# Modalities/modalities

Measured on AMD Instinct MI355X. Metric: train_tokens_per_s, higher is better.
Workload: dtype bf16; 1 GPU; model=gpt2-2.7b, global_batch=2, micro_batch=2, seq_len=4096, parallelism=dp1_fullshard_hipgraph, num_params=2795276800

## Files before the change

### modalities_amd/models/gpt2.py

```python

import math
from enum import Enum
from typing import Annotated, Optional

import torch
import torch.nn as nn
from pydantic import BaseModel, Field, model_validator

from modalities_amd.models.model import NNModel, SwiGLU
from modalities_amd.ops import flash_attention, precompute_rope_cos_sin, rope_apply
from modalities_amd.exceptions import ConfigError
from modalities_amd.ops.attention import (DECODE_HEAD_DIMS, _doc_visible,
                                          decode_attention,
                                          decode_attention_enabled,
                                          decode_rope_append, document_starts,
                                          fused_qkv_rope_attention)
from modalities_amd.ops.backend import use_hip
from modalities_amd.ops.layer_norm import LayerNorm
from modalities_amd.ops.linear import TwoStreamLinear
from modalities_amd.ops.rms_norm import RMSNorm


class PositionTypes(str, Enum):
    ABSOLUTE = "ABSOLUTE"
    NOPE = "NOPE"


class AttentionImplementation(str, Enum):
    HIP_FLASH = "hip_flash"
    PYTORCH_FLASH = "pytorch_flash"
    MANUAL = "manual"


class ActivationType(str, Enum):
    GELU = "gelu"
    SWIGLU = "swiglu"


class QueryKeyValueTransformType(str, Enum):
    ROTARY = "RotaryTransform"
    IDENTITY = "IdentityTransform"


class LayerNormVariant(str, Enum):
    RMS_NORM = "rms_norm"
    LAYER_NORM = "layer_norm"


class LayerNormConfig(BaseModel):
    variant: LayerNormVariant = LayerNormVariant.RMS_NORM
    eps: float = 1e-6
    bias: bool = True

# ... 215 lines not shown
            att = att.masked_fill(~mask, float("-inf")).softmax(-1)
            y = att @ vt
        return y.transpose(1, 2)


class TransformerMLP(nn.Module):
    def __init__(self, n_embd: int, ffn_hidden: int, bias: bool, dropout: float):
        super().__init__()
        self.c_fc = TwoStreamLinear(n_embd, ffn_hidden, bias=bias)
        self.gelu = nn.GELU(approximate="tanh")
        self.c_proj = TwoStreamLinear(ffn_hidden, n_embd, bias=bias)
        self.dropout = nn.Dropout(dropout)

    def forward(self, x):
        return self.dropout(self.c_proj(self.gelu(self.c_fc(x))))


class GPT2Block(nn.Module):

    def __init__(self, cfg: GPT2LLMConfig):
        super().__init__()
        self.attention_norm = make_norm(cfg.attention_norm_config, cfg.n_embd)
        self.attn = CausalSelfAttention(
            cfg.n_embd, cfg.n_head_q, cfg.n_head_kv, cfg.bias, cfg.dropout,
            cfg.attention_implementation, cfg.use_qk_norm,
            cfg.attention_norm_config, fused_qkv=cfg.fused_qkv)
        self.ffn_norm = make_norm(cfg.ffn_norm_config, cfg.n_embd)
        if cfg.activation_type == ActivationType.SWIGLU:
            self.mlp = SwiGLU(cfg.n_embd, cfg.ffn_hidden, cfg.bias,
                              packed=cfg.packed_swiglu)
        else:
            self.mlp = TransformerMLP(cfg.n_embd, cfg.ffn_hidden, cfg.bias, cfg.dropout)

    def forward(self, x, rope_cos, rope_sin, doc_start=None):
        if doc_start is None:
            x = x + self.attn(self.attention_norm(x), rope_cos, rope_sin)
        else:
            x = x + self.attn(self.attention_norm(x), rope_cos, rope_sin,
                              doc_start=doc_start)
        x = x + self.mlp(self.ffn_norm(x))
        return x

    def forward_cached(self, x, rope_cos, rope_sin, cache_k, cache_v, pos,
                       dec=None):
        if dec is None:
            x = x + self.attn.forward_cached(self.attention_norm(x), rope_cos,
                                             rope_sin, cache_k, cache_v, pos)
        else:
            x = x + self.attn.forward_cached(self.attention_norm(x), rope_cos,
                                             rope_sin, cache_k, cache_v, pos,
                                             dec=dec)
        x = x + self.mlp(self.ffn_norm(x))
        return x


class GPT2LLM(NNModel):
    def __init__(self, config: GPT2LLMConfig):
        if isinstance(config, dict):
            config = GPT2LLMConfig(**config)
        weight_decay_groups = {
            "linear": [r"attn\..*attn\.weight", r"attn\.qkv_attn\.weight",
                       r"attn\.c_proj\.weight",
                       r"mlp\..*\.weight", r"lm_head\.weight"],
            "embedding": [r"wte\.weight", r"wpe\.weight"],
            "norm": [r"norm", r"ln_", r"\.bias"],
        }
        super().__init__(seed=config.seed, weight_decay_groups=weight_decay_groups)
# ... 134 lines not shown
```

### modalities_amd/ops/csrc/bindings.cpp

```cpp
#include <torch/extension.h>

std::vector<torch::Tensor> rmsnorm_fwd(torch::Tensor x, torch::Tensor w, double eps);
std::vector<torch::Tensor> rmsnorm_bwd(torch::Tensor dy, torch::Tensor x,
                                       torch::Tensor w, torch::Tensor invrms);
std::vector<torch::Tensor> layernorm_fwd(torch::Tensor x, torch::Tensor w,
                                         c10::optional<torch::Tensor> b,
                                         double eps);
std::vector<torch::Tensor> layernorm_bwd(torch::Tensor dy, torch::Tensor x,
                                         torch::Tensor w, torch::Tensor mean,
                                         torch::Tensor rstd, bool has_bias);
long layernorm_max_h();
torch::Tensor rope_fwd(torch::Tensor x, torch::Tensor cos_t, torch::Tensor sin_t,
                       bool neg);
torch::Tensor rope_fwd_slice(torch::Tensor qkv, torch::Tensor cos_t,
                             torch::Tensor sin_t, long col_off, long Hn,
                             long D, bool neg);
void rope_bwd_slice(torch::Tensor dx, torch::Tensor cos_t, torch::Tensor sin_t,
                    torch::Tensor dqkv, long col_off);
torch::Tensor silu_mul_fwd(torch::Tensor g, torch::Tensor u);
std::vector<torch::Tensor> silu_mul_bwd(torch::Tensor dout, torch::Tensor g,
                                        torch::Tensor u);
torch::Tensor silu_mul_joint_fwd(torch::Tensor wv);
torch::Tensor silu_mul_joint_bwd(torch::Tensor dout, torch::Tensor wv);
std::vector<torch::Tensor> cross_entropy_fwd(torch::Tensor logits,
                                             torch::Tensor targets,
                                             long ignore_index);
torch::Tensor cross_entropy_bwd(torch::Tensor logits, torch::Tensor targets,
                                torch::Tensor lse, torch::Tensor scale,
                                long ignore_index);
void fused_adamw_masked(torch::Tensor p, torch::Tensor g, torch::Tensor m,
                        torch::Tensor v, torch::Tensor wd_mask, double lr,
                        double beta1, double beta2, double eps, double wd,
                        double bc1, double bc2);
void fused_adamw_masked_devstep(torch::Tensor p, torch::Tensor g,
                                torch::Tensor m, torch::Tensor v,
                                torch::Tensor wd_mask, torch::Tensor step,
                                torch::Tensor bf16_out,
// ... 61 lines not shown
                                         torch::Tensor k, torch::Tensor v,
                                         torch::Tensor o, torch::Tensor lse,
                                         bool causal, long q_offset,
                                         torch::Tensor doc_start,
                                         torch::Tensor doc_end,
                                         c10::optional<torch::Tensor> dlse);
std::vector<torch::Tensor> attn_bwd2_qkvjoint_doc(
    torch::Tensor dout, torch::Tensor q, torch::Tensor k, torch::Tensor v,
    torch::Tensor o, torch::Tensor lse, bool causal, long q_offset,
    torch::Tensor doc_start, torch::Tensor doc_end, torch::Tensor dqkv,
    long dv_col_off);
std::vector<torch::Tensor> decode_attn_fwd(torch::Tensor q,
                                           torch::Tensor k_cache,
                                           torch::Tensor v_cache,
                                           torch::Tensor kv_lens,
                                           long kv_chunk);
long decode_attn_kv_chunk();
long decode_attn_kv_chunk_min();
torch::Tensor decode_rope_append(torch::Tensor q, torch::Tensor k,
                                 torch::Tensor v,
                                 c10::optional<torch::Tensor> cos_t,
                                 c10::optional<torch::Tensor> sin_t,
                                 torch::Tensor pos, torch::Tensor k_cache,
                                 torch::Tensor v_cache);

static int g_attn_impl = [] {
  const char* e = getenv("MA_ATTN_IMPL");
  return e ? atoi(e) : 2;
}();

PYBIND11_MODULE(TORCH_EXTENSION_NAME, m) {
  m.def("rmsnorm_fwd", &rmsnorm_fwd, "RMSNorm forward (K5)");
  m.def("rmsnorm_bwd", &rmsnorm_bwd, "RMSNorm backward (K5)");
  m.def("layernorm_fwd", &layernorm_fwd,
        "LayerNorm forward (K5): (y, mean, rstd); b may be None",
        py::arg("x"), py::arg("w"), py::arg("b"), py::arg("eps"));
  m.def("layernorm_bwd", &layernorm_bwd,
        "LayerNorm backward (K5): (dx, dw, db); db is empty without bias",
        py::arg("dy"), py::arg("x"), py::arg("w"), py::arg("mean"),
        py::arg("rstd"), py::arg("has_bias"));
  m.def("layernorm_max_h", &layernorm_max_h,
        "largest row length the LayerNorm kernels take");
  m.def("rope_fwd", &rope_fwd, "RoPE rotate-half (K4); neg=true => inverse");
  m.def("rope_fwd_slice", &rope_fwd_slice,
        "RoPE a head-block slice of fused QKV into a contiguous [B,T,H,D]");
  m.def("rope_bwd_slice", &rope_bwd_slice,
        "inverse-RoPE a [B,T,H,D] grad into a fused-QKV grad buffer slice");
  m.def("silu_mul_fwd", &silu_mul_fwd, "silu(g)*u forward (K6)");
  m.def("silu_mul_bwd", &silu_mul_bwd, "silu(g)*u backward (K6)");
  m.def("silu_mul_joint_fwd", &silu_mul_joint_fwd,
        "silu/mul over a packed [.., 2H] gate|up tensor (K6 joint)");
  m.def("silu_mul_joint_bwd", &silu_mul_joint_bwd,
        "joint-layout silu/mul backward into one dwv buffer");
  m.def("cross_entropy_fwd", &cross_entropy_fwd, "fused CE forward (K8)");
  m.def("cross_entropy_bwd", &cross_entropy_bwd, "fused CE backward (K8)");
  m.def("fused_adamw_masked", &fused_adamw_masked,
        "AdamW on a flat fp32 shard with per-element wd mask (K9)");
  m.def("fused_adamw", &fused_adamw, "multi-tensor AdamW (K9)");
  m.def("fused_adamw_masked_devstep", &fused_adamw_masked_devstep,
        "AdamW with device-resident step counter (hipGraph-safe)");
  m.def("multi_tensor_sqsum", &multi_tensor_sqsum, "sum of squares (K10)");
  m.def("fused_adamw_devstep_bf16g", &fused_adamw_devstep_bf16g,
        "device-step AdamW reading a bf16 grad (* gmul) and a bit-packed "
        "decay mask (K9)");
  m.def("multi_tensor_sqsum_bf16", &multi_tensor_sqsum_bf16,
        "sum of squares of float(bf16) * gmul (K10)");
// ... 126 lines not shown
```

### modalities_amd/ops/csrc/rms_norm.hip

```cpp
#include <torch/extension.h>
#include <ATen/hip/HIPContext.h>
#include "common.h"

namespace {

constexpr int BLOCK = 256;

__global__ void rmsnorm_fwd_kernel(const unsigned short* __restrict__ x,
                                   const unsigned short* __restrict__ w,
                                   unsigned short* __restrict__ y,
                                   float* __restrict__ invrms,
                                   int H, float eps) {
  __shared__ float scratch[BLOCK / WAVE_SIZE];
  const long row = blockIdx.x;
  const unsigned short* xr = x + row * (long)H;
  unsigned short* yr = y + row * (long)H;

  float ss = 0.f;
  const int vecH = (H % 8 == 0) ? H / 8 : 0;
  const shortx8* xv = reinterpret_cast<const shortx8*>(xr);
  for (int i = threadIdx.x; i < vecH; i += BLOCK) {
    shortx8 v = xv[i];
#pragma unroll
    for (int j = 0; j < 8; ++j) {
      float f = bf16_to_f32((unsigned short)v[j]);
      ss += f * f;
    }
  }
  for (int i = vecH * 8 + threadIdx.x; i < H; i += BLOCK) {
    float f = bf16_to_f32(xr[i]);
    ss += f * f;
  }
  ss = block_reduce_sum(ss, scratch);
  const float r = rsqrtf(ss / H + eps);
  if (threadIdx.x == 0) invrms[row] = r;

  const shortx8* wv = reinterpret_cast<const shortx8*>(w);
  shortx8* yv = reinterpret_cast<shortx8*>(yr);
  for (int i = threadIdx.x; i < vecH; i += BLOCK) {
    shortx8 xvv = xv[i], wvv = wv[i], o;
#pragma unroll
    for (int j = 0; j < 8; ++j) {
      float f = bf16_to_f32((unsigned short)xvv[j]) * r *
                bf16_to_f32((unsigned short)wvv[j]);
      o[j] = (short)f32_to_bf16(f);
    }
    yv[i] = o;
  }
  for (int i = vecH * 8 + threadIdx.x; i < H; i += BLOCK) {
    yr[i] = f32_to_bf16(bf16_to_f32(xr[i]) * r * bf16_to_f32(w[i]));
  }
}

template <int SLOTS>
__global__ void rmsnorm_bwd_kernel(const unsigned short* __restrict__ dy,
                                   const unsigned short* __restrict__ x,
                                   const unsigned short* __restrict__ w,
                                   const float* __restrict__ invrms,
                                   unsigned short* __restrict__ dx,
                                   float* __restrict__ dw,
                                   int H, long N, int rows_per_block) {
  extern __shared__ __attribute__((aligned(16))) char smem_raw[];
  float* slab = reinterpret_cast<float*>(smem_raw);
  const int nwaves = blockDim.x / WAVE_SIZE;
  const int lane = threadIdx.x & (WAVE_SIZE - 1);
  const int wid = threadIdx.x / WAVE_SIZE;
  float* my_slab = slab + (long)wid * H;

  const long row0 = (long)blockIdx.x * rows_per_block;
  const long row1 = min(row0 + rows_per_block, N);
  const int vecH = H / 8;

  float dwacc[SLOTS][8];
#pragma unroll
  for (int it = 0; it < SLOTS; ++it)
#pragma unroll
    for (int j = 0; j < 8; ++j) dwacc[it][j] = 0.f;

  const shortx8* wv = reinterpret_cast<const shortx8*>(w);
  for (long row = row0 + wid; row < row1; row += nwaves) {
    const shortx8* xv = reinterpret_cast<const shortx8*>(x + row * (long)H);
    const shortx8* dyv = reinterpret_cast<const shortx8*>(dy + row * (long)H);
    shortx8* dxv = reinterpret_cast<shortx8*>(dx + row * (long)H);
    const float r = invrms[row];

    float dot = 0.f;
#pragma unroll
    for (int it = 0; it < SLOTS; ++it) {
      const int i = lane + it * WAVE_SIZE;
      if (i < vecH) {
        shortx8 xvv = xv[i], dyvv = dyv[i], wvv = wv[i];
#pragma unroll
        for (int j = 0; j < 8; ++j) {
          dot += bf16_to_f32((unsigned short)dyvv[j]) *
                 bf16_to_f32((unsigned short)wvv[j]) *
                 bf16_to_f32((unsigned short)xvv[j]);
        }
      }
    }
    dot = wave_reduce_sum(dot);
    const float k = r * r * r * dot / H;

#pragma unroll
    for (int it = 0; it < SLOTS; ++it) {
      const int i = lane + it * WAVE_SIZE;
      if (i < vecH) {
        shortx8 xvv = xv[i], dyvv = dyv[i], wvv = wv[i], o;
#pragma unroll
        for (int j = 0; j < 8; ++j) {
          float xf = bf16_to_f32((unsigned short)xvv[j]);
          float dyf = bf16_to_f32((unsigned short)dyvv[j]);
          float wf = bf16_to_f32((unsigned short)wvv[j]);
          o[j] = (short)f32_to_bf16(r * wf * dyf - k * xf);
          dwacc[it][j] += dyf * xf * r;
        }
        dxv[i] = o;
      }
    }
  }

#pragma unroll
  for (int it = 0; it < SLOTS; ++it) {
    const int i = lane + it * WAVE_SIZE;
    if (i < vecH)
#pragma unroll
      for (int j = 0; j < 8; ++j) my_slab[i * 8 + j] = dwacc[it][j];
  }
  __syncthreads();
  for (int i = threadIdx.x; i < H; i += blockDim.x) {
    float acc = 0.f;
    for (int sl = 0; sl < nwaves; ++sl) acc += slab[(long)sl * H + i];
    dw[(long)blockIdx.x * H + i] = acc;
  }
}

__global__ void dw_reduce_kernel(const float* __restrict__ dw_part,
                                 float* __restrict__ dw, int H, int nblocks,
                                 int rows_per_chunk) {
  const int i = blockIdx.x * blockDim.x + threadIdx.x;
  if (i >= H) return;
  const int b0 = blockIdx.y * rows_per_chunk;
  const int b1 = min(b0 + rows_per_chunk, nblocks);
  float acc = 0.f;
  for (int b = b0; b < b1; ++b) acc += dw_part[(long)b * H + i];
  if (gridDim.y == 1) dw[i] = acc;
  else atomicAdd(&dw[i], acc);
}

}

std::vector<torch::Tensor> rmsnorm_fwd(torch::Tensor x, torch::Tensor w, double eps) {
  TORCH_CHECK(x.is_cuda() && x.dtype() == torch::kBFloat16, "x must be device bf16");
  TORCH_CHECK(x.dim() == 2 && x.is_contiguous());
  TORCH_CHECK(w.is_cuda() && w.dtype() == torch::kBFloat16
              && w.is_contiguous() && w.numel() == x.size(1),
              "rmsnorm_fwd: w must be contiguous device bf16 [H]");
  const long N = x.size(0);
  const int H = x.size(1);
  auto y = torch::empty_like(x);
  auto invrms = torch::empty({N}, x.options().dtype(torch::kFloat32));
  auto stream = at::cuda::getCurrentHIPStream();
  hipLaunchKernelGGL(rmsnorm_fwd_kernel, dim3(N), dim3(BLOCK), 0, stream,
                     (const unsigned short*)x.data_ptr(),
                     (const unsigned short*)w.data_ptr(),
                     (unsigned short*)y.data_ptr(),
                     invrms.data_ptr<float>(), H, (float)eps);
  HIP_CHECK_KERNEL();
  return {y, invrms};
}

std::vector<torch::Tensor> rmsnorm_bwd(torch::Tensor dy, torch::Tensor x,
                                       torch::Tensor w, torch::Tensor invrms) {
  TORCH_CHECK(x.is_cuda() && x.dtype() == torch::kBFloat16 && x.dim() == 2
              && x.is_contiguous(),
              "rmsnorm_bwd: x must be contiguous device bf16 [N,H]");
  const long N = x.size(0);
  const int H = x.size(1);
  TORCH_CHECK(dy.is_cuda() && dy.dtype() == torch::kBFloat16
              && dy.is_contiguous() && dy.dim() == 2 && dy.size(0) == N
              && dy.size(1) == H,
              "rmsnorm_bwd: dy must be contiguous device bf16 [N,H]");
  TORCH_CHECK(w.is_cuda() && w.dtype() == torch::kBFloat16
              && w.is_contiguous() && w.numel() == H,
              "rmsnorm_bwd: w must be contiguous device bf16 [H]");
  TORCH_CHECK(invrms.is_cuda() && invrms.dtype() == torch::kFloat32
              && invrms.is_contiguous() && invrms.numel() == N,
              "rmsnorm_bwd: invrms must be contiguous device fp32 [N]");
  auto dx = torch::empty_like(x);
  auto dw = torch::zeros({H}, x.options().dtype(torch::kFloat32));
  torch::Tensor dw_part;
  int nblocks = (int)min((long)2048, (N + 3) / 4);
  int rows_per_block = (int)((N + nblocks - 1) / nblocks);
  nblocks = (int)((N + rows_per_block - 1) / rows_per_block);
  const int nwaves = BLOCK / WAVE_SIZE;
  size_t smem = (size_t)H * nwaves * sizeof(float);
  TORCH_CHECK(smem <= 160 * 1024, "rmsnorm_bwd: H too large for LDS slabs");
  TORCH_CHECK(H % 8 == 0, "rmsnorm_bwd: H must be divisible by 8");
  const int slots = (H / 8 + WAVE_SIZE - 1) / WAVE_SIZE;
  dw_part = torch::empty({(long)nblocks, (long)H},
                         x.options().dtype(torch::kFloat32));
  auto stream = at::cuda::getCurrentHIPStream();
  auto launch = [&](auto* kfn) {
    hipLaunchKernelGGL(kfn, dim3(nblocks), dim3(BLOCK), smem, stream,
                       (const unsigned short*)dy.data_ptr(),
                       (const unsigned short*)x.data_ptr(),
                       (const unsigned short*)w.data_ptr(),
                       invrms.data_ptr<float>(),
                       (unsigned short*)dx.data_ptr(),
                       dw_part.data_ptr<float>(), H, N, rows_per_block);
  };
  if (slots <= 1) launch(rmsnorm_bwd_kernel<1>);
  else if (slots <= 2) launch(rmsnorm_bwd_kernel<2>);
  else if (slots <= 5) launch(rmsnorm_bwd_kernel<5>);
  else if (slots <= 8) launch(rmsnorm_bwd_kernel<8>);
  else if (slots <= 16) launch(rmsnorm_bwd_kernel<16>);
  else TORCH_CHECK(false, "rmsnorm_bwd: H too large (max 8192)");
  {
    const int chunks = (int)min((long)32, (long)((nblocks + 63) / 64));
    const int rpc = (nblocks + chunks - 1) / chunks;
    hipLaunchKernelGGL(dw_reduce_kernel,
                       dim3((H + BLOCK - 1) / BLOCK, chunks), dim3(BLOCK), 0,
                       stream, dw_part.data_ptr<float>(),
                       dw.data_ptr<float>(), H, nblocks, rpc);
  }
  HIP_CHECK_KERNEL();
  return {dx, dw};
}
```

### modalities_amd/ops/linear.py

```python

import os
from typing import Optional

import torch
import torch.nn as nn

_side_stream: Optional[torch.cuda.Stream] = None

_TWO_STREAM_MAX_WEIGHT = int(os.environ.get(
    "MODALITIES_AMD_TWO_STREAM_MAX_WEIGHT", 64 * 1024 * 1024))

_TWO_STREAM_MAX_ROWS = int(os.environ.get(
    "MODALITIES_AMD_TWO_STREAM_MAX_ROWS", 8192))


def _get_side_stream() -> torch.cuda.Stream:
    global _side_stream
    if _side_stream is None:
        _side_stream = torch.cuda.Stream()
    return _side_stream


class _TwoStreamLinearFn(torch.autograd.Function):
    @staticmethod
    def forward(ctx, x, weight, bias):
        ctx.save_for_backward(x, weight)
        ctx.has_bias = bias is not None
        return torch.nn.functional.linear(x, weight, bias)

    @staticmethod
    def backward(ctx, dy):
        x, weight = ctx.saved_tensors
        dy2 = dy.reshape(-1, dy.shape[-1])
        x2 = x.reshape(-1, x.shape[-1])
        if not dy.is_cuda or dy2.shape[0] > _TWO_STREAM_MAX_ROWS:
            dw = dy2.t() @ x2
            db = dy2.sum(0) if ctx.has_bias else None
            dx = (dy2 @ weight).view_as(x)
            return dx, dw, db
        main = torch.cuda.current_stream()
        side = _get_side_stream()
        side.wait_stream(main)
        with torch.cuda.stream(side):
            dw = dy2.t() @ x2
            db = dy2.sum(0) if ctx.has_bias else None
        dx = (dy2 @ weight).view_as(x)
        main.wait_stream(side)
        dw.record_stream(main)
        if db is not None:
            db.record_stream(main)
        return dx, dw, db


class TwoStreamLinear(nn.Linear):
    def forward(self, x: torch.Tensor) -> torch.Tensor:
        if x.is_cuda and torch.is_grad_enabled() and (
                x.requires_grad or self.weight.requires_grad) and \
                self.weight.numel() <= _TWO_STREAM_MAX_WEIGHT:
            return _TwoStreamLinearFn.apply(x, self.weight, self.bias)
        return torch.nn.functional.linear(x, self.weight, self.bias)
```

### modalities_amd/ops/rms_norm.py

```python

import torch

from modalities_amd.ops.backend import use_hip, hip_ext


def _rms_norm_ref(x: torch.Tensor, weight: torch.Tensor, eps: float) -> torch.Tensor:
    xf = x.float()
    inv = torch.rsqrt(xf.pow(2).mean(-1, keepdim=True) + eps)
    return (xf * inv * weight.float()).to(x.dtype)


class _RMSNormHip(torch.autograd.Function):
    @staticmethod
    def forward(ctx, x, weight, eps):
        shape = x.shape
        x2d = x.contiguous().view(-1, shape[-1])
        y, invrms = hip_ext().rmsnorm_fwd(x2d, weight, eps)
        ctx.save_for_backward(x2d, weight, invrms)
        ctx.shape = shape
        return y.view(shape)

    @staticmethod
    def backward(ctx, dy):
        x2d, weight, invrms = ctx.saved_tensors
        dx, dw = hip_ext().rmsnorm_bwd(dy.contiguous().view_as(x2d), x2d, weight, invrms)
        return dx.view(ctx.shape), dw.to(weight.dtype), None


def rms_norm(x: torch.Tensor, weight: torch.Tensor, eps: float = 1e-6) -> torch.Tensor:
    if use_hip(x, weight):
        return _RMSNormHip.apply(x, weight, eps)
    return _rms_norm_ref(x, weight, eps)


class RMSNorm(torch.nn.Module):

    def __init__(self, normalized_shape: int, eps: float = 1e-6, device=None, dtype=None):
        super().__init__()
        self.eps = eps
        self.normalized_shape = normalized_shape
        self.weight = torch.nn.Parameter(
            torch.empty(normalized_shape, device=device, dtype=dtype))
        self.reset_parameters()

    def reset_parameters(self):
        torch.nn.init.ones_(self.weight)

    def forward(self, x: torch.Tensor) -> torch.Tensor:
        return rms_norm(x, self.weight, self.eps)

    def extra_repr(self):
        return f"{self.normalized_shape}, eps={self.eps}"
```

### modalities_amd/parallel/fsdp.py

```python

import os
import re
from contextlib import contextmanager
from typing import Optional

import torch
import torch.distributed as dist
import torch.nn as nn


def _pad_to(n: int, multiple: int) -> int:
    return (n + multiple - 1) // multiple * multiple


class _CommStreams:
    def __init__(self, device: torch.device):
        self.on_gpu = device.type == "cuda"
        self.gather = torch.cuda.Stream(device=device) if self.on_gpu else None
        self.reduce = torch.cuda.Stream(device=device) if self.on_gpu else None

    @contextmanager
    def on(self, stream):
        if self.on_gpu and stream is not None:
            with torch.cuda.stream(stream):
                yield
        else:
            yield


class FlatParamUnit:

    def __init__(self, name: str, modules: list[nn.Module], device: torch.device,
                 group, rank: int, world: int, param_dtype: torch.dtype,
                 no_decay_patterns: Optional[list[str]] = None):
        self.name = name
        self.modules = modules
        self.device = device
        self.group = group
        self.rank = rank
        self.world = world
        self.param_dtype = param_dtype
# ... 9 lines not shown

        self.shapes = [p.shape for _, _, p in self.param_infos]
        self.numels = [p.numel() for _, _, p in self.param_infos]
        self.offsets = []
        off = 0
        for n in self.numels:
            self.offsets.append(off)
            off += n
        self.total_numel = _pad_to(max(off, 1), max(world, 1) * 64)
        self.shard_numel = self.total_numel // world

        nd_res = [re.compile(pat) for pat in (no_decay_patterns or [])]
        flat_mask = torch.ones(self.total_numel, dtype=torch.float32)
        for (mod, pname, p), offset, numel in zip(self.param_infos, self.offsets,
                                                  self.numels):
            full_name = f"{type(mod).__name__}.{pname}"
            no_decay = p.ndim < 2 or any(r.search(full_name) for r in nd_res)
            if no_decay:
                flat_mask[offset:offset + numel] = 0.0
        s = self.rank * self.shard_numel
        self.wd_mask_shard = flat_mask[s:s + self.shard_numel].to(device)

        self.master_shard = torch.zeros(self.shard_numel, dtype=torch.float32, device=device)
        self._grad_shard_f32 = torch.empty(self.shard_numel, dtype=torch.float32,
                                           device=device)
        self.grad_fresh = False
        self.keep_bf16_grads = (
            device.type == "cuda" and param_dtype == torch.bfloat16
            and os.environ.get("MODALITIES_AMD_BF16_GRAD_PATH", "1") != "0")
        self._pending_grad: Optional[torch.Tensor] = None
        self._pending_gmul = 1.0
        self.bf16_shard = torch.zeros(self.shard_numel, dtype=param_dtype, device=device)
        self.full_buf: Optional[torch.Tensor] = None
        self.grad_full: Optional[torch.Tensor] = None
        self.is_gathered = False
        self.grads_allocated = False
        self.grads_seen = 0
        self._gather_event = None
        self._reduce_event = None


    @property
    def grad_shard(self) -> torch.Tensor:
        self.materialize_grad()
        return self._grad_shard_f32

    @grad_shard.setter
    def grad_shard(self, value: torch.Tensor):
        self._pending_grad = None
        self._grad_shard_f32 = value

    @torch.no_grad()
    def materialize_grad(self):
        out = self._pending_grad
        if out is None:
            return
        self._pending_grad = None
        self._grad_shard_f32.copy_(out)
        if self._pending_gmul != 1.0:
            self._grad_shard_f32.mul_(self._pending_gmul)


    @torch.no_grad()
    def init_from_materialized(self):
        flat = torch.zeros(self.total_numel, dtype=torch.float32, device=self.device)
        for (_, _, p), off, n in zip(self.param_infos, self.offsets, self.numels):
# ... 20 lines not shown
        if self.world == 1:
            self.full_buf = self.bf16_shard
            self.is_gathered = True
            return
        with streams.on(streams.gather):
            if streams.on_gpu:
                streams.gather.wait_stream(torch.cuda.current_stream(self.device))
            self.full_buf = torch.empty(self.total_numel, dtype=self.param_dtype,
                                        device=self.device)
            dist.all_gather_into_tensor(self.full_buf, self.bf16_shard, group=self.group)
            if streams.on_gpu:
                self._gather_event = torch.cuda.Event()
                self._gather_event.record(streams.gather)
        self.is_gathered = True

    def wait_gather(self, streams: _CommStreams):
        if streams.on_gpu and self._gather_event is not None:
            torch.cuda.current_stream(self.device).wait_event(self._gather_event)
            self._gather_event = None
            if self.full_buf is not None and self.full_buf.is_cuda:
                self.full_buf.record_stream(
                    torch.cuda.current_stream(self.device))
        self._point_params_to(self.full_buf)

    @torch.no_grad()
    def free_full(self):
        self._point_params_to(None)
        self.full_buf = None
        self.is_gathered = False


    @torch.no_grad()
    def alloc_grad_views(self):
        if self.grad_full is None:
            self.grad_full = torch.zeros(self.total_numel, dtype=self.param_dtype,
                                         device=self.device)
        for (_, _, p), off, n, shape in zip(self.param_infos, self.offsets,
                                            self.numels, self.shapes):
            p.grad = self.grad_full[off:off + n].view(shape)
        self.grads_allocated = True

    def reduce_scatter_grads(self, streams: _CommStreams):
        gf = self.grad_full
        if gf is None:
            return
        compute = torch.cuda.current_stream(self.device) if streams.on_gpu \
            else None
        with streams.on(streams.reduce):
            if streams.on_gpu:
                streams.reduce.wait_stream(torch.cuda.current_stream(self.device))
            if self.world > 1:
                backend = dist.get_backend(self.group) if self.group is not None \
                    else dist.get_backend()
                if backend != "gloo":
                    out = torch.empty(self.shard_numel, dtype=self.param_dtype,
                                      device=self.device)
                    dist.reduce_scatter_tensor(out, gf, group=self.group)
                else:
                    dist.all_reduce(gf, group=self.group)
                    s = self.rank * self.shard_numel
                    out = gf[s:s + self.shard_numel]
            else:
                out = gf
            scale = 1.0 / self.world
            if self.grad_fresh:
                self.grad_shard.add_(out, alpha=scale)
            else:
                self._pending_grad, self._pending_gmul = out, scale
                if self.keep_bf16_grads:
                    if out is not gf:
                        out.record_stream(compute)
                else:
                    self.materialize_grad()
                self.grad_fresh = True
            if streams.on_gpu:
                self._reduce_event = torch.cuda.Event()
                self._reduce_event.record(streams.reduce)
                gf.record_stream(streams.reduce)
        for _, _, p in self.param_infos:
            p.grad = None
        self.grad_full = None
        self.grads_allocated = False

    def wait_reduce(self):
        if self._reduce_event is not None:
            torch.cuda.current_stream(self.device).wait_event(self._reduce_event)
            self._reduce_event = None

    @torch.no_grad()
    def publish_master(self):
        self.bf16_shard.copy_(self.master_shard)
        if self.world > 1 and self.full_buf is not None:
            self.free_full()


class _UnshardBackwardAnchor(torch.autograd.Function):

    @staticmethod
    def forward(ctx, engine, unit_idx, t):
        ctx.engine = engine
        ctx.unit_idx = unit_idx
        return t.view_as(t)

    @staticmethod
    def backward(ctx, grad):
        ctx.engine._pre_backward(ctx.unit_idx)
        return None, None, grad


class XGMIShardedModel(nn.Module):

    def __init__(self, module: nn.Module, device: torch.device,
                 process_group=None, rank: Optional[int] = None,
                 world_size: Optional[int] = None,
# ... 35 lines not shown
            u.init_from_materialized()

    @staticmethod
    def from_transformer(model, device, process_group=None, blocks_per_unit: int = 1,
                         reshard_after_forward: bool = False,
                         param_dtype: torch.dtype = torch.bfloat16,
                         no_decay_patterns: Optional[list[str]] = None,
                         rank=None, world_size=None,
                         replicate_group=None) -> "XGMIShardedModel":
        blocks = list(model.blocks)
        unit_modules = [blocks[i:i + blocks_per_unit]
                        for i in range(0, len(blocks), blocks_per_unit)]
        root_mods = [m for name, m in model.named_children() if name != "blocks"]
        unit_modules.append(root_mods)
        return XGMIShardedModel(model, device, process_group=process_group,
                                unit_modules=unit_modules, param_dtype=param_dtype,
                                reshard_after_forward=reshard_after_forward,
                                no_decay_patterns=no_decay_patterns,
                                rank=rank, world_size=world_size,
                                replicate_group=replicate_group)


    def _install_hooks(self, unit_modules: list[list[nn.Module]]):
        for idx, mods in enumerate(unit_modules):
            for m in mods:
                if not any(True for _ in m.parameters(recurse=True)):
                    continue
                m.register_forward_pre_hook(self._make_fwd_pre(idx))
                m.register_forward_hook(self._make_fwd_post(idx))

    def _install_grad_hooks(self):
        for idx, unit in enumerate(self.units):
            expected = len(unit.param_infos)
            for _, _, p in unit.param_infos:
                p.register_post_accumulate_grad_hook(
                    self._make_grad_hook(idx, expected))

    def _make_grad_hook(self, idx, expected):
        def hook(param):
            unit = self.units[idx]
            unit.grads_seen += 1
            if unit.grads_seen >= expected:
                unit.grads_seen = 0
                self._finish_unit_backward(idx)
        return hook

    def _wrap(self, fn, idx, obj):
        if isinstance(obj, torch.Tensor) and obj.is_floating_point() and obj.requires_grad:
            return fn.apply(self, idx, obj)
        if isinstance(obj, tuple):
            return tuple(self._wrap(fn, idx, o) for o in obj)
        return obj

    def _make_fwd_pre(self, idx):
        def hook(module, args):
            unit = self.units[idx]
            if not unit.is_gathered:
                unit.gather(self.streams)
            unit.wait_gather(self.streams)
            if idx not in self._fwd_order:
                self._fwd_order.append(idx)
                self._prefetch_after(idx)
            if torch.is_grad_enabled():
                self._units_needing_reduce.add(idx)
            return args
        return hook

    def _make_fwd_post(self, idx):
        def hook(module, args, output):
            if torch.is_grad_enabled():
                output = self._wrap(_UnshardBackwardAnchor, idx, output)
            if self.reshard_after_forward and torch.is_grad_enabled():
                unit = self.units[idx]
# ... 164 lines not shown
```

Before: 36110 tokens/s.

## Fuse residual add into RMSNorm and write weight grads into FSDP slots

```diff
diff --git a/modalities_amd/models/gpt2.py b/modalities_amd/models/gpt2.py
--- a/modalities_amd/models/gpt2.py
+++ b/modalities_amd/models/gpt2.py
@@ -1,5 +1,6 @@
 
 import math
+import os
 from enum import Enum
 from typing import Annotated, Optional
 
@@ -18,7 +19,7 @@
 from modalities_amd.ops.backend import use_hip
 from modalities_amd.ops.layer_norm import LayerNorm
 from modalities_amd.ops.linear import TwoStreamLinear
-from modalities_amd.ops.rms_norm import RMSNorm
+from modalities_amd.ops.rms_norm import RMSNorm, add_rms_norm
 
 
 class PositionTypes(str, Enum):
@@ -300,7 +301,23 @@
         else:
             self.mlp = TransformerMLP(cfg.n_embd, cfg.ffn_hidden, cfg.bias, cfg.dropout)
 
+    def _fused_norms(self, x) -> bool:
+        an, fn = self.attention_norm, self.ffn_norm
+        return (type(an) is RMSNorm and type(fn) is RMSNorm
+                and os.environ.get("MODALITIES_AMD_FUSED_ADD_NORM", "1") != "0"
+                and x.dtype == torch.bfloat16
+                and use_hip(x, an.weight, fn.weight))
+
     def forward(self, x, rope_cos, rope_sin, doc_start=None):
+        if self._fused_norms(x):
+            an, fn = self.attention_norm, self.ffn_norm
+            h0, y1 = add_rms_norm(x, None, an.weight, an.eps)
+            if doc_start is None:
+                a = self.attn(y1, rope_cos, rope_sin)
+            else:
+                a = self.attn(y1, rope_cos, rope_sin, doc_start=doc_start)
+            h1, y2 = add_rms_norm(h0, a, fn.weight, fn.eps)
+            return h1 + self.mlp(y2)
         if doc_start is None:
             x = x + self.attn(self.attention_norm(x), rope_cos, rope_sin)
         else:
diff --git a/modalities_amd/ops/csrc/bindings.cpp b/modalities_amd/ops/csrc/bindings.cpp
--- a/modalities_amd/ops/csrc/bindings.cpp
+++ b/modalities_amd/ops/csrc/bindings.cpp
@@ -3,6 +3,11 @@
 std::vector<torch::Tensor> rmsnorm_fwd(torch::Tensor x, torch::Tensor w, double eps);
 std::vector<torch::Tensor> rmsnorm_bwd(torch::Tensor dy, torch::Tensor x,
                                        torch::Tensor w, torch::Tensor invrms);
+std::vector<torch::Tensor> add_rmsnorm_fwd(torch::Tensor x, torch::Tensor r,
+                                           torch::Tensor w, double eps);
+std::vector<torch::Tensor> rmsnorm_bwd_fused(
+    torch::Tensor dy, torch::Tensor x, torch::Tensor w, torch::Tensor invrms,
+    c10::optional<torch::Tensor> g, c10::optional<torch::Tensor> dw_out);
 std::vector<torch::Tensor> layernorm_fwd(torch::Tensor x, torch::Tensor w,
                                          c10::optional<torch::Tensor> b,
                                          double eps);
@@ -130,6 +135,13 @@
 PYBIND11_MODULE(TORCH_EXTENSION_NAME, m) {
   m.def("rmsnorm_fwd", &rmsnorm_fwd, "RMSNorm forward (K5)");
   m.def("rmsnorm_bwd", &rmsnorm_bwd, "RMSNorm backward (K5)");
+  m.def("add_rmsnorm_fwd", &add_rmsnorm_fwd,
+        "Residual add + RMSNorm forward (K5): (h, y, invrms), h = x + r");
+  m.def("rmsnorm_bwd_fused", &rmsnorm_bwd_fused,
+        "RMSNorm backward (K5) with dx += g and dw merged deterministically "
+        "into dw_out (bf16 [H]) or a fresh fp32 [H]; g, dw_out may be None",
+        py::arg("dy"), py::arg("x"), py::arg("w"), py::arg("invrms"),
+        py::arg("g"), py::arg("dw_out"));
   m.def("layernorm_fwd", &layernorm_fwd,
         "LayerNorm forward (K5): (y, mean, rstd); b may be None",
         py::arg("x"), py::arg("w"), py::arg("b"), py::arg("eps"));
diff --git a/modalities_amd/ops/csrc/rms_norm.hip b/modalities_amd/ops/csrc/rms_norm.hip
--- a/modalities_amd/ops/csrc/rms_norm.hip
+++ b/modalities_amd/ops/csrc/rms_norm.hip
@@ -52,11 +52,117 @@
   }
 }
 
-template <int SLOTS>
+template <int VPT>
+__global__ void add_rmsnorm_fwd_kernel(const unsigned short* __restrict__ x,
+                                       const unsigned short* __restrict__ res,
+                                       const unsigned short* __restrict__ w,
+                                       unsigned short* __restrict__ h,
+                                       unsigned short* __restrict__ y,
+                                       float* __restrict__ invrms,
+                                       int H, float eps) {
+  __shared__ float scratch[BLOCK / WAVE_SIZE];
+  const long row = blockIdx.x;
+  const unsigned short* xr = x + row * (long)H;
+  const unsigned short* rr = res + row * (long)H;
+  unsigned short* hr = h + row * (long)H;
+  unsigned short* yr = y + row * (long)H;
+  const shortx8* wv = reinterpret_cast<const shortx8*>(w);
+  shortx8* yv = reinterpret_cast<shortx8*>(yr);
+
+  float ss = 0.f;
+  if (VPT > 0) {
+    const int vecH = H / 8;
+    const shortx8* xv = reinterpret_cast<const shortx8*>(xr);
+    const shortx8* rv = reinterpret_cast<const shortx8*>(rr);
+    shortx8* hv = reinterpret_cast<shortx8*>(hr);
+    shortx8 hreg[VPT > 0 ? VPT : 1];
+#pragma unroll
+    for (int it = 0; it < VPT; ++it) {
+      const int i = threadIdx.x + it * BLOCK;
+      if (i < vecH) {
+        shortx8 a = xv[i], b = rv[i], o;
+#pragma unroll
+        for (int j = 0; j < 8; ++j) {
+          unsigned short s = f32_to_bf16(bf16_to_f32((unsigned short)a[j]) +
+                                         bf16_to_f32((unsigned short)b[j]));
+          o[j] = (short)s;
+          float f = bf16_to_f32(s);
+          ss += f * f;
+        }
+        hv[i] = o;
+        hreg[it] = o;
+      }
+    }
+    ss = block_reduce_sum(ss, scratch);
+    const float r = rsqrtf(ss / H + eps);
+    if (threadIdx.x == 0) invrms[row] = r;
+#pragma unroll
+    for (int it = 0; it < VPT; ++it) {
+      const int i = threadIdx.x + it * BLOCK;
+      if (i < vecH) {
+        shortx8 hvv = hreg[it], wvv = wv[i], o;
+#pragma unroll
+        for (int j = 0; j < 8; ++j) {
+          float f = bf16_to_f32((unsigned short)hvv[j]) * r *
+                    bf16_to_f32((unsigned short)wvv[j]);
+          o[j] = (short)f32_to_bf16(f);
+        }
+        yv[i] = o;
+      }
+    }
+    return;
+  }
+
+  const int vecH = (H % 8 == 0) ? H / 8 : 0;
+  {
+    const shortx8* xv = reinterpret_cast<const shortx8*>(xr);
+    const shortx8* rv = reinterpret_cast<const shortx8*>(rr);
+    shortx8* hv = reinterpret_cast<shortx8*>(hr);
+    for (int i = threadIdx.x; i < vecH; i += BLOCK) {
+      shortx8 a = xv[i], b = rv[i], o;
+#pragma unroll
+      for (int j = 0; j < 8; ++j) {
+        unsigned short s = f32_to_bf16(bf16_to_f32((unsigned short)a[j]) +
+                                       bf16_to_f32((unsigned short)b[j]));
+        o[j] = (short)s;
+        float f = bf16_to_f32(s);
+        ss += f * f;
+      }
+      hv[i] = o;
+    }
+  }
+  for (int i = vecH * 8 + threadIdx.x; i < H; i += BLOCK) {
+    unsigned short s = f32_to_bf16(bf16_to_f32(xr[i]) + bf16_to_f32(rr[i]));
+    hr[i] = s;
+    float f = bf16_to_f32(s);
+    ss += f * f;
+  }
+  ss = block_reduce_sum(ss, scratch);
+  const float r = rsqrtf(ss / H + eps);
+  if (threadIdx.x == 0) invrms[row] = r;
+
+  const shortx8* hv = reinterpret_cast<const shortx8*>(hr);
+  for (int i = threadIdx.x; i < vecH; i += BLOCK) {
+    shortx8 hvv = hv[i], wvv = wv[i], o;
+#pragma unroll
+    for (int j = 0; j < 8; ++j) {
+      float f = bf16_to_f32((unsigned short)hvv[j]) * r *
+                bf16_to_f32((unsigned short)wvv[j]);
+      o[j] = (short)f32_to_bf16(f);
+    }
+    yv[i] = o;
+  }
+  for (int i = vecH * 8 + threadIdx.x; i < H; i += BLOCK) {
+    yr[i] = f32_to_bf16(bf16_to_f32(hr[i]) * r * bf16_to_f32(w[i]));
+  }
+}
+
+template <int SLOTS, bool HAS_G>
 __global__ void rmsnorm_bwd_kernel(const unsigned short* __restrict__ dy,
                                    const unsigned short* __restrict__ x,
                                    const unsigned short* __restrict__ w,
                                    const float* __restrict__ invrms,
+                                   const unsigned short* __restrict__ g,
                                    unsigned short* __restrict__ dx,
                                    float* __restrict__ dw,
                                    int H, long N, int rows_per_block) {
@@ -82,6 +188,8 @@
     const shortx8* xv = reinterpret_cast<const shortx8*>(x + row * (long)H);
     const shortx8* dyv = reinterpret_cast<const shortx8*>(dy + row * (long)H);
     shortx8* dxv = reinterpret_cast<shortx8*>(dx + row * (long)H);
+    const shortx8* gv = HAS_G
+        ? reinterpret_cast<const shortx8*>(g + row * (long)H) : nullptr;
     const float r = invrms[row];
 
     float dot = 0.f;
@@ -105,13 +213,18 @@
     for (int it = 0; it < SLOTS; ++it) {
       const int i = lane + it * WAVE_SIZE;
       if (i < vecH) {
-        shortx8 xvv = xv[i], dyvv = dyv[i], wvv = wv[i], o;
+        shortx8 xvv = xv[i], dyvv = dyv[i], wvv = wv[i], gvv, o;
+        if (HAS_G) gvv = gv[i];
 #pragma unroll
         for (int j = 0; j < 8; ++j) {
           float xf = bf16_to_f32((unsigned short)xvv[j]);
           float dyf = bf16_to_f32((unsigned short)dyvv[j]);
           float wf = bf16_to_f32((unsigned short)wvv[j]);
-          o[j] = (short)f32_to_bf16(r * wf * dyf - k * xf);
+          unsigned short d = f32_to_bf16(r * wf * dyf - k * xf);
+          if (HAS_G)
+            d = f32_to_bf16(bf16_to_f32(d) +
+                            bf16_to_f32((unsigned short)gvv[j]));
+          o[j] = (short)d;
           dwacc[it][j] += dyf * xf * r;
         }
         dxv[i] = o;
@@ -145,6 +258,96 @@
   for (int b = b0; b < b1; ++b) acc += dw_part[(long)b * H + i];
   if (gridDim.y == 1) dw[i] = acc;
   else atomicAdd(&dw[i], acc);
+}
+
+constexpr int FIN_COLS = 16;
+constexpr int FIN_ROWS = 64;
+
+__device__ __forceinline__ void store_dw(float* p, float v) { *p = v; }
+__device__ __forceinline__ void store_dw(unsigned short* p, float v) {
+  *p = f32_to_bf16(v);
+}
+
+template <typename out_t>
+__global__ void __launch_bounds__(FIN_COLS * FIN_ROWS) dw_finish_kernel(const float* __restrict__ dw_part,
+                                 out_t* __restrict__ dw, int H, int nblocks) {
+  __shared__ float part[FIN_ROWS][FIN_COLS];
+  const int c = threadIdx.x % FIN_COLS;
+  const int rl = threadIdx.x / FIN_COLS;
+  const int col = blockIdx.x * FIN_COLS + c;
+  float acc = 0.f;
+  if (col < H) {
+#pragma unroll 4
+    for (int b = rl; b < nblocks; b += FIN_ROWS)
+      acc += dw_part[(long)b * H + col];
+  }
+  part[rl][c] = acc;
+  __syncthreads();
+  if (rl == 0 && col < H) {
+    float total = 0.f;
+#pragma unroll 8
+    for (int i = 0; i < FIN_ROWS; ++i) total += part[i][c];
+    store_dw(dw + col, total);
+  }
+}
+
+torch::Tensor launch_rmsnorm_bwd(const torch::Tensor& dy, const torch::Tensor& x,
+                                 const torch::Tensor& w,
+                                 const torch::Tensor& invrms,
+                                 const unsigned short* g, torch::Tensor& dx,
+                                 const char* name) {
+  TORCH_CHECK(x.is_cuda() && x.dtype() == torch::kBFloat16 && x.dim() == 2
+              && x.is_contiguous(),
+              name, ": x must be contiguous device bf16 [N,H]");
+  const long N = x.size(0);
+  const int H = x.size(1);
+  TORCH_CHECK(dy.is_cuda() && dy.dtype() == torch::kBFloat16
+              && dy.is_contiguous() && dy.dim() == 2 && dy.size(0) == N
+              && dy.size(1) == H,
+              name, ": dy must be contiguous device bf16 [N,H]");
+  TORCH_CHECK(w.is_cuda() && w.dtype() == torch::kBFloat16
+              && w.is_contiguous() && w.numel() == H,
+              name, ": w must be contiguous device bf16 [H]");
+  TORCH_CHECK(invrms.is_cuda() && invrms.dtype() == torch::kFloat32
+              && invrms.is_contiguous() && invrms.numel() == N,
+              name, ": invrms must be contiguous device fp32 [N]");
+  TORCH_CHECK(N > 0, name, ": empty input");
+  int nblocks = (int)min((long)2048, (N + 3) / 4);
+  int rows_per_block = (int)((N + nblocks - 1) / nblocks);
+  nblocks = (int)((N + rows_per_block - 1) / rows_per_block);
+  const int nwaves = BLOCK / WAVE_SIZE;
+  size_t smem = (size_t)H * nwaves * sizeof(float);
+  TORCH_CHECK(smem <= 160 * 1024, name, ": H too large for LDS slabs");
+  TORCH_CHECK(H % 8 == 0, name, ": H must be divisible by 8");
+  const int slots = (H / 8 + WAVE_SIZE - 1) / WAVE_SIZE;
+  TORCH_CHECK(slots <= 16, name, ": H too large (max 8192)");
+  dx = torch::empty_like(x);
+  auto dw_part = torch::empty({(long)nblocks, (long)H},
+                              x.options().dtype(torch::kFloat32));
+  auto stream = at::cuda::getCurrentHIPStream();
+  auto launch = [&](auto* kfn) {
+    hipLaunchKernelGGL(kfn, dim3(nblocks), dim3(BLOCK), smem, stream,
+                       (const unsigned short*)dy.data_ptr(),
+                       (const unsigned short*)x.data_ptr(),
+                       (const unsigned short*)w.data_ptr(),
+                       invrms.data_ptr<float>(), g,
+                       (unsigned short*)dx.data_ptr(),
+                       dw_part.data_ptr<float>(), H, N, rows_per_block);
+  };
+  if (g == nullptr) {
+    if (slots <= 1) launch(rmsnorm_bwd_kernel<1, false>);
+    else if (slots <= 2) launch(rmsnorm_bwd_kernel<2, false>);
+    else if (slots <= 5) launch(rmsnorm_bwd_kernel<5, false>);
+    else if (slots <= 8) launch(rmsnorm_bwd_kernel<8, false>);
+    else launch(rmsnorm_bwd_kernel<16, false>);
+  } else {
+    if (slots <= 1) launch(rmsnorm_bwd_kernel<1, true>);
+    else if (slots <= 2) launch(rmsnorm_bwd_kernel<2, true>);
+    else if (slots <= 5) launch(rmsnorm_bwd_kernel<5, true>);
+    else if (slots <= 8) launch(rmsnorm_bwd_kernel<8, true>);
+    else launch(rmsnorm_bwd_kernel<16, true>);
+  }
+  return dw_part;
 }
 
 }
@@ -169,60 +372,99 @@
   return {y, invrms};
 }
 
+std::vector<torch::Tensor> add_rmsnorm_fwd(torch::Tensor x, torch::Tensor r,
+                                           torch::Tensor w, double eps) {
+  TORCH_CHECK(x.is_cuda() && x.dtype() == torch::kBFloat16 && x.dim() == 2
+              && x.is_contiguous(),
+              "add_rmsnorm_fwd: x must be contiguous device bf16 [N,H]");
+  TORCH_CHECK(r.is_cuda() && r.dtype() == torch::kBFloat16 && r.dim() == 2
+              && r.is_contiguous() && r.size(0) == x.size(0)
+              && r.size(1) == x.size(1),
+              "add_rmsnorm_fwd: r must be contiguous device bf16 [N,H]");
+  TORCH_CHECK(w.is_cuda() && w.dtype() == torch::kBFloat16
+              && w.is_contiguous() && w.numel() == x.size(1),
+              "add_rmsnorm_fwd: w must be contiguous device bf16 [H]");
+  const long N = x.size(0);
+  const int H = x.size(1);
+  auto h = torch::empty_like(x);
+  auto y = torch::empty_like(x);
+  auto invrms = torch::empty({N}, x.options().dtype(torch::kFloat32));
+  if (N == 0) return {h, y, invrms};
+  auto stream = at::cuda::getCurrentHIPStream();
+  auto launch = [&](auto* kfn) {
+    hipLaunchKernelGGL(kfn, dim3(N), dim3(BLOCK), 0, stream,
+                       (const unsigned short*)x.data_ptr(),
+                       (const unsigned short*)r.data_ptr(),
+                       (const unsigned short*)w.data_ptr(),
+                       (unsigned short*)h.data_ptr(),
+                       (unsigned short*)y.data_ptr(),
+                       invrms.data_ptr<float>(), H, (float)eps);
+  };
+  const int vec_per_thread = (H % 8 == 0) ? (H / 8 + BLOCK - 1) / BLOCK : 0;
+  if (vec_per_thread == 1) launch(add_rmsnorm_fwd_kernel<1>);
+  else if (vec_per_thread == 2) launch(add_rmsnorm_fwd_kernel<2>);
+  else if (vec_per_thread >= 3 && vec_per_thread <= 4)
+    launch(add_rmsnorm_fwd_kernel<4>);
+  else launch(add_rmsnorm_fwd_kernel<0>);
+  HIP_CHECK_KERNEL();
+  return {h, y, invrms};
+}
+
 std::vector<torch::Tensor> rmsnorm_bwd(torch::Tensor dy, torch::Tensor x,
                                        torch::Tensor w, torch::Tensor invrms) {
-  TORCH_CHECK(x.is_cuda() && x.dtype() == torch::kBFloat16 && x.dim() == 2
-              && x.is_contiguous(),
-              "rmsnorm_bwd: x must be contiguous device bf16 [N,H]");
-  const long N = x.size(0);
+  torch::Tensor dx;
+  auto dw_part = launch_rmsnorm_bwd(dy, x, w, invrms, nullptr, dx,
+                                    "rmsnorm_bwd");
   const int H = x.size(1);
-  TORCH_CHECK(dy.is_cuda() && dy.dtype() == torch::kBFloat16
-              && dy.is_contiguous() && dy.dim() == 2 && dy.size(0) == N
-              && dy.size(1) == H,
-              "rmsnorm_bwd: dy must be contiguous device bf16 [N,H]");
-  TORCH_CHECK(w.is_cuda() && w.dtype() == torch::kBFloat16
-              && w.is_contiguous() && w.numel() == H,
-              "rmsnorm_bwd: w must be contiguous device bf16 [H]");
-  TORCH_CHECK(invrms.is_cuda() && invrms.dtype() == torch::kFloat32
-              && invrms.is_contiguous() && invrms.numel() == N,
-              "rmsnorm_bwd: invrms must be contiguous device fp32 [N]");
-  auto dx = torch::empty_like(x);
+  const int nblocks = dw_part.size(0);
   auto dw = torch::zeros({H}, x.options().dtype(torch::kFloat32));
-  torch::Tensor dw_part;
-  int nblocks = (int)min((long)2048, (N + 3) / 4);
-  int rows_per_block = (int)((N + nblocks - 1) / nblocks);
-  nblocks = (int)((N + rows_per_block - 1) / rows_per_block);
-  const int nwaves = BLOCK / WAVE_SIZE;
-  size_t smem = (size_t)H * nwaves * sizeof(float);
-  TORCH_CHECK(smem <= 160 * 1024, "rmsnorm_bwd: H too large for LDS slabs");
-  TORCH_CHECK(H % 8 == 0, "rmsnorm_bwd: H must be divisible by 8");
-  const int slots = (H / 8 + WAVE_SIZE - 1) / WAVE_SIZE;
-  dw_part = torch::empty({(long)nblocks, (long)H},
-                         x.options().dtype(torch::kFloat32));
-  auto stream = at::cuda::getCurrentHIPStream();
-  auto launch = [&](auto* kfn) {
-    hipLaunchKernelGGL(kfn, dim3(nblocks), dim3(BLOCK), smem, stream,
-                       (const unsigned short*)dy.data_ptr(),
-                       (const unsigned short*)x.data_ptr(),
-                       (const unsigned short*)w.data_ptr(),
-                       invrms.data_ptr<float>(),
-                       (unsigned short*)dx.data_ptr(),
-                       dw_part.data_ptr<float>(), H, N, rows_per_block);
-  };
-  if (slots <= 1) launch(rmsnorm_bwd_kernel<1>);
-  else if (slots <= 2) launch(rmsnorm_bwd_kernel<2>);
-  else if (slots <= 5) launch(rmsnorm_bwd_kernel<5>);
-  else if (slots <= 8) launch(rmsnorm_bwd_kernel<8>);
-  else if (slots <= 16) launch(rmsnorm_bwd_kernel<16>);
-  else TORCH_CHECK(false, "rmsnorm_bwd: H too large (max 8192)");
-  {
-    const int chunks = (int)min((long)32, (long)((nblocks + 63) / 64));
-    const int rpc = (nblocks + chunks - 1) / chunks;
-    hipLaunchKernelGGL(dw_reduce_kernel,
-                       dim3((H + BLOCK - 1) / BLOCK, chunks), dim3(BLOCK), 0,
-                       stream, dw_part.data_ptr<float>(),
-                       dw.data_ptr<float>(), H, nblocks, rpc);
-  }
+  const int chunks = (int)min((long)32, (long)((nblocks + 63) / 64));
+  const int rpc = (nblocks + chunks - 1) / chunks;
+  hipLaunchKernelGGL(dw_reduce_kernel,
+                     dim3((H + BLOCK - 1) / BLOCK, chunks), dim3(BLOCK), 0,
+                     at::cuda::getCurrentHIPStream(),
+                     dw_part.data_ptr<float>(), dw.data_ptr<float>(), H,
+                     nblocks, rpc);
   HIP_CHECK_KERNEL();
   return {dx, dw};
 }
+
+std::vector<torch::Tensor> rmsnorm_bwd_fused(
+    torch::Tensor dy, torch::Tensor x, torch::Tensor w, torch::Tensor invrms,
+    c10::optional<torch::Tensor> g, c10::optional<torch::Tensor> dw_out) {
+  const unsigned short* gp = nullptr;
+  if (g.has_value()) {
+    TORCH_CHECK(g->is_cuda() && g->dtype() == torch::kBFloat16
+                && g->is_contiguous() && g->dim() == 2 && x.dim() == 2
+                && g->size(0) == x.size(0) && g->size(1) == x.size(1),
+                "rmsnorm_bwd_fused: g must be contiguous device bf16 [N,H]");
+    gp = (const unsigned short*)g->data_ptr();
+  }
+  if (dw_out.has_value()) {
+    TORCH_CHECK(dw_out->is_cuda() && dw_out->dtype() == torch::kBFloat16
+                && dw_out->is_contiguous() && dw_out->dim() == 1
+                && dw_out->numel() == w.numel(),
+                "rmsnorm_bwd_fused: dw_out must be contiguous device bf16 [H]");
+  }
+  torch::Tensor dx;
+  auto dw_part = launch_rmsnorm_bwd(dy, x, w, invrms, gp, dx,
+                                    "rmsnorm_bwd_fused");
+  const int H = x.size(1);
+  const int nblocks = dw_part.size(0);
+  const dim3 grid((H + FIN_COLS - 1) / FIN_COLS), block(FIN_COLS * FIN_ROWS);
+  auto stream = at::cuda::getCurrentHIPStream();
+  torch::Tensor dw;
+  if (dw_out.has_value()) {
+    dw = *dw_out;
+    hipLaunchKernelGGL(dw_finish_kernel<unsigned short>, grid, block, 0,
+                       stream, dw_part.data_ptr<float>(),
+                       (unsigned short*)dw.data_ptr(), H, nblocks);
+  } else {
+    dw = torch::empty({H}, x.options().dtype(torch::kFloat32));
+    hipLaunchKernelGGL(dw_finish_kernel<float>, grid, block, 0, stream,
+                       dw_part.data_ptr<float>(), dw.data_ptr<float>(), H,
+                       nblocks);
+  }
+  HIP_CHECK_KERNEL();
+  return {dx, dw};
+}
diff --git a/modalities_amd/ops/grad_slot.py b/modalities_amd/ops/grad_slot.py
--- /dev/null
+++ b/modalities_amd/ops/grad_slot.py
@@ -0,0 +1,27 @@
+
+import os
+from typing import Callable, Optional
+
+import torch
+
+_ATTR = "_flat_grad_slot"
+
+
+def inplace_wgrad_enabled() -> bool:
+    return os.environ.get("MODALITIES_AMD_INPLACE_WGRAD", "1") != "0"
+
+
+def tag_param(param: torch.nn.Parameter,
+              claim: Callable[..., Optional[torch.Tensor]]) -> None:
+    setattr(param, _ATTR, claim)
+
+
+def slot_of(param: torch.Tensor) -> Optional[Callable[..., Optional[torch.Tensor]]]:
+    return getattr(param, _ATTR, None)
+
+
+def claim(slot: Optional[Callable[..., Optional[torch.Tensor]]],
+          like: torch.Tensor) -> Optional[torch.Tensor]:
+    if slot is None:
+        return None
+    return slot(like.dtype, like.device)
diff --git a/modalities_amd/ops/linear.py b/modalities_amd/ops/linear.py
--- a/modalities_amd/ops/linear.py
+++ b/modalities_amd/ops/linear.py
@@ -4,6 +4,8 @@
 
 import torch
 import torch.nn as nn
+
+from modalities_amd.ops import grad_slot
 
 _side_stream: Optional[torch.cuda.Stream] = None
 
@@ -22,28 +24,46 @@
 
 
 class _TwoStreamLinearFn(torch.autograd.Function):
+
     @staticmethod
     def forward(ctx, x, weight, bias):
         ctx.save_for_backward(x, weight)
         ctx.has_bias = bias is not None
+        ctx.w_slot = grad_slot.slot_of(weight)
+        ctx.b_slot = grad_slot.slot_of(bias) if bias is not None else None
         return torch.nn.functional.linear(x, weight, bias)
+
+    @staticmethod
+    def _wgrad(ctx, dy2, x2):
+        dw = grad_slot.claim(ctx.w_slot, dy2)
+        if dw is None:
+            dw = dy2.t() @ x2
+        else:
+            torch.mm(dy2.t(), x2, out=dw)
+        db = None
+        if ctx.has_bias:
+            db = grad_slot.claim(ctx.b_slot, dy2)
+            if db is None:
+                db = dy2.sum(0)
+            else:
+                torch.sum(dy2, 0, out=db)
+        return dw, db
 
     @staticmethod
     def backward(ctx, dy):
         x, weight = ctx.saved_tensors
         dy2 = dy.reshape(-1, dy.shape[-1])
         x2 = x.reshape(-1, x.shape[-1])
-        if not dy.is_cuda or dy2.shape[0] > _TWO_STREAM_MAX_ROWS:
-            dw = dy2.t() @ x2
-            db = dy2.sum(0) if ctx.has_bias else None
+        if not dy.is_cuda or dy2.shape[0] > _TWO_STREAM_MAX_ROWS \
+                or weight.numel() > _TWO_STREAM_MAX_WEIGHT:
+            dw, db = _TwoStreamLinearFn._wgrad(ctx, dy2, x2)
             dx = (dy2 @ weight).view_as(x)
             return dx, dw, db
         main = torch.cuda.current_stream()
         side = _get_side_stream()
         side.wait_stream(main)
         with torch.cuda.stream(side):
-            dw = dy2.t() @ x2
-            db = dy2.sum(0) if ctx.has_bias else None
+            dw, db = _TwoStreamLinearFn._wgrad(ctx, dy2, x2)
         dx = (dy2 @ weight).view_as(x)
         main.wait_stream(side)
         dw.record_stream(main)
@@ -54,8 +74,8 @@
 
 class TwoStreamLinear(nn.Linear):
     def forward(self, x: torch.Tensor) -> torch.Tensor:
-        if x.is_cuda and torch.is_grad_enabled() and (
-                x.requires_grad or self.weight.requires_grad) and \
-                self.weight.numel() <= _TWO_STREAM_MAX_WEIGHT:
+        if torch.is_grad_enabled() and (
+                x.requires_grad or self.weight.requires_grad) and (
+                x.is_cuda or grad_slot.slot_of(self.weight) is not None):
             return _TwoStreamLinearFn.apply(x, self.weight, self.bias)
         return torch.nn.functional.linear(x, self.weight, self.bias)
diff --git a/modalities_amd/ops/rms_norm.py b/modalities_amd/ops/rms_norm.py
--- a/modalities_amd/ops/rms_norm.py
+++ b/modalities_amd/ops/rms_norm.py
@@ -1,6 +1,7 @@
 
 import torch
 
+from modalities_amd.ops import grad_slot
 from modalities_amd.ops.backend import use_hip, hip_ext
 
 
@@ -27,6 +28,45 @@
         return dx.view(ctx.shape), dw.to(weight.dtype), None
 
 
+class _AddRMSNormHip(torch.autograd.Function):
+
+    @staticmethod
+    def forward(ctx, x, r, weight, eps):
+        shape = x.shape
+        x2d = x.contiguous().view(-1, shape[-1])
+        if r is None:
+            y, invrms = hip_ext().rmsnorm_fwd(x2d, weight, eps)
+            h, h2d = x, x2d
+        else:
+            h2d, y, invrms = hip_ext().add_rmsnorm_fwd(
+                x2d, r.contiguous().view(-1, shape[-1]), weight, eps)
+            h = h2d.view(shape)
+        ctx.save_for_backward(h2d, weight, invrms)
+        ctx.shape = shape
+        ctx.has_r = r is not None
+        ctx.w_slot = grad_slot.slot_of(weight)
+        ctx.set_materialize_grads(False)
+        return h, y.view(shape)
+
+    @staticmethod
+    def backward(ctx, g_h, dy):
+        if dy is None:
+            return g_h, (g_h if ctx.has_r else None), None, None
+        h2d, weight, invrms = ctx.saved_tensors
+        g = None if g_h is None else g_h.contiguous().view_as(h2d)
+        dy2d = dy.contiguous().view_as(h2d)
+        dx, dw = hip_ext().rmsnorm_bwd_fused(
+            dy2d, h2d, weight, invrms, g, grad_slot.claim(ctx.w_slot, dy2d))
+        if dw.dtype != weight.dtype:
+            dw = dw.to(weight.dtype)
+        dx = dx.view(ctx.shape)
+        return dx, (dx if ctx.has_r else None), dw, None
+
+
+def add_rms_norm(x: torch.Tensor, r, weight: torch.Tensor, eps: float = 1e-6):
+    return _AddRMSNormHip.apply(x, r, weight, eps)
+
+
 def rms_norm(x: torch.Tensor, weight: torch.Tensor, eps: float = 1e-6) -> torch.Tensor:
     if use_hip(x, weight):
         return _RMSNormHip.apply(x, weight, eps)
diff --git a/modalities_amd/parallel/fsdp.py b/modalities_amd/parallel/fsdp.py
--- a/modalities_amd/parallel/fsdp.py
+++ b/modalities_amd/parallel/fsdp.py
@@ -1,4 +1,5 @@
 
+import functools
 import os
 import re
 from contextlib import contextmanager
@@ -7,6 +8,8 @@
 import torch
 import torch.distributed as dist
 import torch.nn as nn
+
+from modalities_amd.ops import grad_slot
 
 
 def _pad_to(n: int, multiple: int) -> int:
@@ -82,6 +85,12 @@
         self._pending_gmul = 1.0
         self.bf16_shard = torch.zeros(self.shard_numel, dtype=param_dtype, device=device)
         self.full_buf: Optional[torch.Tensor] = None
+        self.inplace_wgrad = grad_slot.inplace_wgrad_enabled()
+        self._slot_claimed: list[bool] = []
+        self._slot_written: list[bool] = []
+        if self.inplace_wgrad:
+            for i, (_, _, p) in enumerate(self.param_infos):
+                grad_slot.tag_param(p, functools.partial(self.claim_grad_slot, i))
         self.grad_full: Optional[torch.Tensor] = None
         self.is_gathered = False
         self.grads_allocated = False
@@ -168,19 +177,66 @@
 
     @torch.no_grad()
     def alloc_grad_views(self):
+        if not self.inplace_wgrad:
+            if self.grad_full is None:
+                self.grad_full = torch.zeros(self.total_numel,
+                                             dtype=self.param_dtype,
+                                             device=self.device)
+            for (_, _, p), off, n, shape in zip(self.param_infos, self.offsets,
+                                                self.numels, self.shapes):
+                p.grad = self.grad_full[off:off + n].view(shape)
+            self.grads_allocated = True
+            return
         if self.grad_full is None:
-            self.grad_full = torch.zeros(self.total_numel, dtype=self.param_dtype,
+            self.grad_full = torch.empty(self.total_numel, dtype=self.param_dtype,
                                          device=self.device)
-        for (_, _, p), off, n, shape in zip(self.param_infos, self.offsets,
-                                            self.numels, self.shapes):
-            p.grad = self.grad_full[off:off + n].view(shape)
+            used = self.offsets[-1] + self.numels[-1] if self.numels else 0
+            if used < self.total_numel:
+                self.grad_full[used:].zero_()
+            self._slot_claimed = [False] * len(self.param_infos)
+            self._slot_written = [False] * len(self.param_infos)
         self.grads_allocated = True
+
+    def _slot_view(self, i: int) -> torch.Tensor:
+        off, n = self.offsets[i], self.numels[i]
+        return self.grad_full[off:off + n].view(self.shapes[i])
+
+    def claim_grad_slot(self, i: int, dtype: torch.dtype,
+                        device: torch.device) -> Optional[torch.Tensor]:
+        if self.grad_full is None or self._slot_claimed[i] \
+                or dtype != self.param_dtype \
+                or device != self.grad_full.device:
+            return None
+        self._slot_claimed[i] = True
+        return self._slot_view(i)
+
+    @torch.no_grad()
+    def adopt_grad(self, i: int, p: nn.Parameter):
+        if self.grad_full is None or p.grad is None:
+            return
+        self._slot_written[i] = True
+        itemsize = self.grad_full.element_size()
+        slot_ptr = self.grad_full.data_ptr() + self.offsets[i] * itemsize
+        if p.grad.data_ptr() == slot_ptr and p.grad.dtype == self.param_dtype:
+            return
+        slot = self._slot_view(i)
+        slot.copy_(p.grad)
+        p.grad = slot
+
+    @torch.no_grad()
+    def zero_unwritten_slots(self):
+        if self.grad_full is None or not self.inplace_wgrad:
+            return
+        for i, written in enumerate(self._slot_written):
+            if not written:
+                self._slot_view(i).zero_()
 
     def reduce_scatter_grads(self, streams: _CommStreams):
         gf = self.grad_full
         if gf is None:
             return
-        compute = torch.cuda.current_stream(self.device) if streams.on_gpu \
+        self.zero_unwritten_slots()
+        compute =torch.cuda.current_stream(self.device) if streams.on_gpu \
             else None
         with streams.on(streams.reduce):
             if streams.on_gpu:
@@ -216,6 +272,8 @@
         for _, _, p in self.param_infos:
             p.grad = None
         self.grad_full = None
+        self._slot_claimed = []
+        self._slot_written = []
         self.grads_allocated = False
 
     def wait_reduce(self):
@@ -317,13 +375,15 @@
     def _install_grad_hooks(self):
         for idx, unit in enumerate(self.units):
             expected = len(unit.param_infos)
-            for _, _, p in unit.param_infos:
+            for i, (_, _, p) in enumerate(unit.param_infos):
                 p.register_post_accumulate_grad_hook(
-                    self._make_grad_hook(idx, expected))
-
-    def _make_grad_hook(self, idx, expected):
+                    self._make_grad_hook(idx, expected, i))
+
+    def _make_grad_hook(self, idx, expected, i):
         def hook(param):
             unit = self.units[idx]
+            if unit.inplace_wgrad:
+                unit.adopt_grad(i, param)
             unit.grads_seen += 1
             if unit.grads_seen >= expected:
                 unit.grads_seen = 0
```

Result: no change. 36360 tokens/s (median of 6 runs) (+0.7%).
